# caizexin/GenVC

Measured on AMD Instinct MI355X. Metric: utterances/s (streaming, 1 s chunks; with RTF and first-chunk latency), higher is better.
Workload: dtype f32; 1 GPU; GenVC_small streaming, 1 s chunks, top_k=1, batch 1 per GPU (BASELINE configs[1]); parallelism=replicas x1, utterances sharded by rank, all_gather of token ids

## Files before the change

genvc_amd/csrc/gemm.h:

```cpp
#pragma once
#include "common.h"

namespace gvc {

__host__ __device__ __forceinline__ size_t fm16_index(int m, int k, int K) {
    return ((size_t)(m >> 4) * (K >> 4) + (k >> 4)) * 256 + (size_t)((((m & 15) + 16 * ((k & 15) >> 2)) << 2) + (k & 3));
}

enum GemmAct { ACT_NONE = 0, ACT_GELU_NEW = 1, ACT_RELU = 2, ACT_GELU_ERF = 3 };
enum GemmAAct { AACT_NONE = 0, AACT_LRELU = 1 };

struct GemmEpi {
    const float* bias;
    long long bias_batch_stride;
    int act;
    const float* resid;
    int ldr;
    long long resid_batch_stride;
    long long resid_batch_stride2;
    int resid_fm16;
    int geglu;
    const float* resid2;
    float out_scale;
    int c_fm16;
    int qkv;
    int d, n_head, head_dim, max_seq, T;
    float* kcache; float* vcache;
    int kv_bf16;
    const int32_t* slots;
    const int32_t* base_len;
};

struct GemmArgs {
    const float* A; int lda; long long a_batch_stride;
    const float* Wt; int ldw; long long w_batch_stride;
    int w_bf16;
    float* C; int ldc; long long c_batch_stride;
    int batch_inner; long long a_batch_stride2, c_batch_stride2;
    int M, N, K;
    int conv_cin, conv_tap_stride;
    int a_act; float a_slope;
    const float* att_part; int att_nc, att_heads, att_hd;
    int SK;
    float* work;
    GemmEpi e;
};

__device__ __forceinline__ long long gemm_boff(const GemmArgs& G, int batch, long long s1, long long s2) {
    return G.batch_inner > 0 ? (long long)(batch % G.batch_inner) * s1 + (long long)(batch / G.batch_inner) * s2 : (long long)batch * s1;
}
__device__ __forceinline__ int gemm_binner(const GemmArgs& G, int batch) { return G.batch_inner > 0 ? batch % G.batch_inner : batch; }

__device__ __forceinline__ void gemm_store_nb(const GemmArgs& G, int batch, int m, int n, float v) {
    const GemmEpi& e = G.e;
    if (e.act == ACT_GELU_NEW) v = gelu_new(v);
    else if (e.act == ACT_RELU) v = fmaxf(v, 0.f);
    else if (e.act == ACT_GELU_ERF) v = gelu_erf(v);
    if (e.qkv) {
        const int which = n / e.d;
        const int c = n - which * e.d;
        if (which == 0) {
            G.C[(size_t)m * G.ldc + c] = v;
        } else {
            const int b = m / e.T, t = m - b * e.T;
            const int slot = e.slots[b];
            const int pos = t + (e.base_len ? e.base_len[slot] : 0);
            const int h = c / e.head_dim, j = c - h * e.head_dim;
            float* cache = which == 1 ? e.kcache : e.vcache;
            const size_t at = (((size_t)slot * e.n_head + h) * e.max_seq + pos) * e.head_dim + j;
            if (e.kv_bf16) reinterpret_cast<unsigned short*>(cache)[at] = f32_to_bf16(v);
            else cache[at] = v;
        }
        return;
    }
    if (e.resid) v += e.resid[gemm_boff(G, batch, e.resid_batch_stride, e.resid_batch_stride2) + (size_t)m * e.ldr + n];
    if (e.resid2) v += e.resid2[gemm_boff(G, batch, e.resid_batch_stride, e.resid_batch_stride2) + (size_t)m * e.ldr + n];
    if (e.out_scale != 0.f) v *= e.out_scale;
    if (e.c_fm16) { G.C[fm16_index(m, n, G.N)] = v; return; }
    G.C[gemm_boff(G, batch, G.c_batch_stride, G.c_batch_stride2) + (size_t)m * G.ldc + n] = v;
}

__device__ __forceinline__ void gemm_store(const GemmArgs& G, int batch, int m, int n, float v) {
    if (G.e.bias) v += G.e.bias[gemm_binner(G, batch) * G.e.bias_batch_stride + n];
    gemm_store_nb(G, batch, m, n, v);
}

__device__ __forceinline__ void gemm_store4(const GemmArgs& G, int m, int n, float4 v) {
    const GemmEpi& e = G.e;
    if (e.bias) {
        const float4 b = *reinterpret_cast<const float4*>(e.bias + n);
        v.x += b.x; v.y += b.y; v.z += b.z; v.w += b.w;
    }
    if (e.act == ACT_GELU_NEW) { v.x = gelu_new(v.x); v.y = gelu_new(v.y); v.z = gelu_new(v.z); v.w = gelu_new(v.w); }
    else if (e.act == ACT_RELU) { v.x = fmaxf(v.x, 0.f); v.y = fmaxf(v.y, 0.f); v.z = fmaxf(v.z, 0.f); v.w = fmaxf(v.w, 0.f); }
    else if (e.act == ACT_GELU_ERF) { v.x = gelu_erf(v.x); v.y = gelu_erf(v.y); v.z = gelu_erf(v.z); v.w = gelu_erf(v.w); }
    if (e.qkv) {
        const int which = n / e.d;
        const int c = n - which * e.d;
        if (which == 0) {
            *reinterpret_cast<float4*>(G.C + (size_t)m * G.ldc + c) = v;
        } else {
            const int b = m / e.T, t = m - b * e.T;
            const int slot = e.slots[b];
            const int pos = t + (e.base_len ? e.base_len[slot] : 0);
            const int h = c / e.head_dim, j = c - h * e.head_dim;
            float* cache = which == 1 ? e.kcache : e.vcache;
            const size_t at = (((size_t)slot * e.n_head + h) * e.max_seq + pos) * e.head_dim + j;
            if (e.kv_bf16) {
                ushort4 o;
                o.x = f32_to_bf16(v.x); o.y = f32_to_bf16(v.y); o.z = f32_to_bf16(v.z); o.w = f32_to_bf16(v.w);
                *reinterpret_cast<ushort4*>(reinterpret_cast<unsigned short*>(cache) + at) = o;
// ... 128 lines not shown
```

genvc_amd/csrc/gpt.hip:

```cpp
#include <stdlib.h>

#include <map>
#include <string>
#include <tuple>
#include <vector>

#include "gemm.h"
#include <algorithm>
#include "gpt_kernels.h"
#include "persist_kernel.h"
#include "persist_rows.h"
#include "persist_rows_b16.h"
#include "beam.h"
#include "cfg.h"
#include "contrastive.h"
#include "sampler.h"
#include "seqscore.h"
#include "spec.h"

namespace gvc {

__global__ void k_ln_rows(const float* src, float* dst, int rows, int d, const float* w1, const float* b1,
                          const float* w2, const float* b2, int dst_fm16) {
    const int lane = threadIdx.x & 63;
// ... 1 lines not shown
    if (row >= rows) return;
    const float* x = src + (size_t)row * d;
    float* y = dst + (size_t)row * d;
    const float inv_d = 1.0f / (float)d;
    for (int pass = 0; pass < (w2 ? 2 : 1); ++pass) {
        const float* in = pass == 0 ? x : y;
        const float* gw = pass == 0 ? w1 : w2;
        const float* gb = pass == 0 ? b1 : b2;
        float s = 0.f;
        for (int k = lane * 4; k < d; k += 256) {
            const float4 v = *reinterpret_cast<const float4*>(in + k);
            s += (v.x + v.y) + (v.z + v.w);
        }
        const float mean = wave_sum(s) * inv_d;
        float q = 0.f;
        for (int k = lane * 4; k < d; k += 256) {
            const float4 v = *reinterpret_cast<const float4*>(in + k);
            const float a0 = v.x - mean, a1 = v.y - mean, a2 = v.z - mean, a3 = v.w - mean;
            q += (a0 * a0 + a1 * a1) + (a2 * a2 + a3 * a3);
        }
        const float rstd = 1.0f / sqrtf(wave_sum(q) * inv_d + 1e-5f);
        for (int k = lane * 4; k < d; k += 256) {
            float4 v = *reinterpret_cast<const float4*>(in + k);
            const float4 g = *reinterpret_cast<const float4*>(gw + k);
            const float4 c = *reinterpret_cast<const float4*>(gb + k);
            v.x = (v.x - mean) * rstd * g.x + c.x; v.y = (v.y - mean) * rstd * g.y + c.y;
            v.z = (v.z - mean) * rstd * g.z + c.z; v.w = (v.w - mean) * rstd * g.w + c.w;
            if (dst_fm16 && !w2) *reinterpret_cast<float4*>(dst + fm16_index(row, k, d)) = v;
            else *reinterpret_cast<float4*>(y + k) = v;
        }
    }
}

__global__ void k_embed_rows(float* x, const float* prefix_emb, int B, int T, int P, int d, const float* mel_emb,
                             const float* mel_pos, const int32_t* codes, int n, int start_tok, int stop_tok, int t_off) {
    const int row = blockIdx.x;
    const int Tn = T - t_off;
    const int b = row / Tn, t = row - b * Tn + t_off;
    float* dst = x + (size_t)row * d;
    if (t < P) {
        const float* src = prefix_emb + ((size_t)b * P + t) * d;
        for (int k = threadIdx.x * 4; k < d; k += blockDim.x * 4)
            *reinterpret_cast<float4*>(dst + k) = *reinterpret_cast<const float4*>(src + k);
    } else {
        const int i = t - P;
        const int tok = i == 0 ? start_tok : (i <= n ? codes[(size_t)b * n + i - 1] : stop_tok);
        const float* e = mel_emb + (size_t)tok * d;
        const float* p = mel_pos + (size_t)i * d;
        for (int k = threadIdx.x * 4; k < d; k += blockDim.x * 4) {
            const float4 a = *reinterpret_cast<const float4*>(e + k);
            const float4 c = *reinterpret_cast<const float4*>(p + k);
            *reinterpret_cast<float4*>(dst + k) = make_float4(a.x + c.x, a.y + c.y, a.z + c.z, a.w + c.w);
        }
    }
}

__global__ void k_prefix_rows(float* out, const float* cond, int n_cond, const int32_t* codes, int B, int Tc,
                              int d, const float* text_emb, const float* text_pos, int start_text,
                              int stop_text) {
    const int P = n_cond + Tc + 2;
    const int row = blockIdx.x;
    const int b = row / P, t = row - b * P;
    float* dst = out + (size_t)row * d;
    if (t < n_cond) {
        const float* src = cond + ((size_t)b * n_cond + t) * d;
        for (int k = threadIdx.x * 4; k < d; k += blockDim.x * 4)
            *reinterpret_cast<float4*>(dst + k) = *reinterpret_cast<const float4*>(src + k);
    } else {
        const int i = t - n_cond;
        const int id = i == 0 ? start_text : (i <= Tc ? codes[(size_t)b * Tc + i - 1] : stop_text);
        const float* e = text_emb + (size_t)id * d;
        const float* p = text_pos + (size_t)i * d;
        for (int k = threadIdx.x * 4; k < d; k += blockDim.x * 4) {
            const float4 a = *reinterpret_cast<const float4*>(e + k);
            const float4 c = *reinterpret_cast<const float4*>(p + k);
            *reinterpret_cast<float4*>(dst + k) = make_float4(a.x + c.x, a.y + c.y, a.z + c.z, a.w + c.w);
        }
    }
}

__global__ void k_embed_decode_rows(float* x, const int32_t* tok, const int32_t* slots, GptState st, const float* mel_emb,
                                    const float* mel_pos, int d, int vocab) {
    const int b = blockIdx.x;
    const float* e = mel_emb + (size_t)min(max(tok[b], 0), vocab - 1) * d;
    const float* p = mel_pos + (size_t)st.mel_pos[slots[b]] * d;
    float* dst = x + (size_t)b * d;
    for (int k = threadIdx.x * 4; k < d; k += blockDim.x * 4) {
        const float4 a = *reinterpret_cast<const float4*>(e + k);
        const float4 c = *reinterpret_cast<const float4*>(p + k);
        *reinterpret_cast<float4*>(dst + k) = make_float4(a.x + c.x, a.y + c.y, a.z + c.z, a.w + c.w);
    }
}

__global__ void k_stage_rows(float* stage, float* store, const int32_t* slots, int n, int to_store) {
    const int b = blockIdx.x;
    float* a = stage + (size_t)b * n;
    float* s = store + (size_t)slots[b] * n;
    for (int i = threadIdx.x; i < n; i += blockDim.x) {
        if (to_store) s[i] = a[i];
        else a[i] = s[i];
    }
}

__global__ void k_set_state(GptState st, const int32_t* slots, int B, int seq_len, int mel_pos) {
    const int b = blockIdx.x * blockDim.x + threadIdx.x;
    if (b < B) {
        st.seq_len[slots[b]] = seq_len;
        st.mel_pos[slots[b]] = mel_pos;
        st.pending[slots[b]] = -1;
    }
}

__global__ void k_gather_rows(const float* src, float* dst, int B, int T, int off, int n, int d) {
    const int row = blockIdx.x;
    const int b = row / n, i = row - b * n;
    const float* s = src + ((size_t)b * T + off + i) * d;
    float* o = dst + (size_t)row * d;
    for (int k = threadIdx.x * 4; k < d; k += blockDim.x * 4)
        *reinterpret_cast<float4*>(o + k) = *reinterpret_cast<const float4*>(s + k);
}

__global__ void k_round_bf16(float* w, unsigned short* out, size_t n) {
    for (size_t i = (size_t)blockIdx.x * blockDim.x + threadIdx.x; i < n; i += (size_t)gridDim.x * blockDim.x) {
        const unsigned u = __float_as_uint(w[i]);
        const unsigned r = u + 0x7fffu + ((u >> 16) & 1u);
        out[i] = (unsigned short)(r >> 16);
        w[i] = __uint_as_float(r & 0xffff0000u);
    }
}

__global__ void k_transpose(const float* src, float* dst, int K, int N) {
    __shared__ float tile[32][33];
    const int k0 = blockIdx.y * 32, n0 = blockIdx.x * 32;
    for (int r = threadIdx.y; r < 32; r += blockDim.y) {
        const int k = k0 + r, n = n0 + threadIdx.x;
        if (k < K && n < N) tile[r][threadIdx.x] = src[(size_t)k * N + n];
    }
    __syncthreads();
    for (int r = threadIdx.y; r < 32; r += blockDim.y) {
        const int n = n0 + r, k = k0 + threadIdx.x;
        if (k < K && n < N) dst[(size_t)n * K + k] = tile[threadIdx.x][r];
    }
}
// ... 1260 lines not shown
        G.A = c->h; G.lda = 4 * d; G.Wt = fm ? ly.p2_f : ly.p2_w; G.w_bf16 = fm && c->bf16; G.ldw = 4 * d; G.C = c->x; G.ldc = d; G.M = rows; G.N = d; G.K = 4 * d;
        if (fm) {
            G.work = part_p2;
            if ((rc = gemm_fm(G, strip ? 8 : SKP, 1, &sk_p2))) return rc;
        } else {
            G.work = c->work; G.e.bias = ly.p2_b; G.e.resid = c->x; G.e.ldr = d;
            if ((rc = launch_gemm_cap(G, 1, c->work_cap, s))) return rc;
        }
    }
    if (fm) {
        ln_sum_sk(part_p2, sk_p2, c->layers[c->dm.n_layer - 1].p2_b, nullptr, nullptr);
        GVC_LAUNCH_CHECK();
    }
    return ln_rc;
}

extern "C" int gvc_gpt_prefill(gvc_gpt* c, const int32_t* slots, int32_t B, const float* prefix_emb, int32_t P,
                               int32_t start_tok, float* logits_out, float* latent_out, gvc_stream sv) {
    return gvc_gpt_prefill_cached(c, slots, B, prefix_emb, P, 0, start_tok, logits_out, latent_out, sv);
}

static int prefill_impl(gvc_gpt* c, const int32_t* slots, int32_t B, const float* prefix_emb, int32_t P, int32_t n_cached,
                        int32_t start_tok, float* logits_out, float* latent_out, float* hidden_out, gvc_stream sv) {
    int rc = check_ready(c);
    if (rc) return rc;
    const int T = P + 1, d = c->dm.d_model;
    GVC_REQUIRE(n_cached >= 0 && n_cached <= P, GVC_ERR_ARG, "prefill: n_cached=%d outside [0,%d]", n_cached, P);
    GVC_REQUIRE(B >= 1 && B <= c->dm.max_slots, GVC_ERR_ARG, "prefill: B=%d outside [1,%d]", B, c->dm.max_slots);
    GVC_REQUIRE(P >= 0 && B * T <= c->dm.max_rows, GVC_ERR_ARG, "prefill: %d rows exceed max_rows %d", B * T, c->dm.max_rows);
    GVC_REQUIRE(T < c->dm.max_seq, GVC_ERR_ARG, "prefill: %d rows exceed max_seq %d", T, c->dm.max_seq);
    hipStream_t s = (hipStream_t)sv;
    if (!logits_out) logits_out = c->logits;
    if (!latent_out) latent_out = c->latent;
    hipLaunchKernelGGL(k_embed_rows, dim3(B * (T - n_cached)), dim3(256), 0, s, c->x, prefix_emb, B, T, P, d, c->mel_emb, c->mel_pos,
                       (const int32_t*)nullptr, 0, start_tok, start_tok, n_cached);
    GVC_LAUNCH_CHECK();
    const int Tn = T - n_cached;
    if (n_cached > 0 && rows_persist_ok(c, B * Tn, c->st.seq_len) && (rc = rows_persist_prepare(c))) return rc;
    c->rows_keys_hint = T;
    if (n_cached > 0) {
        hipLaunchKernelGGL(k_set_state, dim3(cdiv(B, 64)), dim3(64), 0, s, c->st, slots, B, n_cached, 0);
        GVC_LAUNCH_CHECK();
        if ((rc = run_rows(c, slots, B, Tn, s, c->st.seq_len))) return rc;
    } else if ((rc = run_rows(c, slots, B, T, s))) return rc;
    if (hidden_out) {
        hipLaunchKernelGGL(k_ln_rows, dim3(cdiv(B * Tn, 4)), dim3(256), 0, s, c->x, hidden_out, B * Tn, d, c->lnf_w, c->lnf_b,
                           (const float*)nullptr, (const float*)nullptr, 0);
        GVC_LAUNCH_CHECK();
    }
    if ((rc = launch_head(c, slots, B, 0, c->x, Tn, Tn - 1, logits_out, latent_out, 0, nullptr, s))) return rc;
    hipLaunchKernelGGL(k_set_state, dim3(cdiv(B, 64)), dim3(64), 0, s, c->st, slots, B, T, 1);
    GVC_LAUNCH_CHECK();
    hipLaunchKernelGGL(k_stage_rows, dim3(B), dim3(256), 0, s, logits_out, c->slot_logits, slots, c->dm.vocab, 1);
    hipLaunchKernelGGL(k_stage_rows, dim3(B), dim3(256), 0, s, latent_out, c->slot_latent, slots, d, 1);
    GVC_LAUNCH_CHECK();
    return GVC_OK;
}

extern "C" int gvc_gpt_prefill_cached(gvc_gpt* c, const int32_t* slots, int32_t B, const float* prefix_emb, int32_t P,
                                      int32_t n_cached, int32_t start_tok, float* logits_out, float* latent_out, gvc_stream sv) {
    return prefill_impl(c, slots, B, prefix_emb, P, n_cached, start_tok, logits_out, latent_out, nullptr, sv);
}

extern "C" int gvc_gpt_prefill_hidden(gvc_gpt* c, const int32_t* slots, int32_t B, const float* prefix_emb, int32_t P, int32_t start_tok,
                                      float* hidden_out, gvc_stream sv) {
    GVC_REQUIRE(hidden_out, GVC_ERR_ARG, "prefill_hidden: null hidden_out");
    return prefill_impl(c, slots, B, prefix_emb, P, 0, start_tok, nullptr, nullptr, hidden_out, sv);
}

extern "C" int gvc_gpt_prefill_cond(gvc_gpt* c, const int32_t* slots, int32_t B, const float* cond_latents, int32_t n_cond, gvc_stream sv) {
    int rc = check_ready(c);
    if (rc) return rc;
    const int d = c->dm.d_model;
    GVC_REQUIRE(B >= 1 && B <= c->dm.max_slots && n_cond >= 1 && B * n_cond <= c->dm.max_rows && n_cond < c->dm.max_seq, GVC_ERR_ARG,
                "prefill_cond: bad B=%d n_cond=%d", B, n_cond);
    hipStream_t s = (hipStream_t)sv;
    hipLaunchKernelGGL(k_embed_rows, dim3(B * n_cond), dim3(256), 0, s, c->x, cond_latents, B, n_cond, n_cond, d, c->mel_emb, c->mel_pos,
                       (const int32_t*)nullptr, 0, 0, 0, 0);
    GVC_LAUNCH_CHECK();
    c->rows_keys_hint = n_cond;
    if ((rc = run_rows(c, slots, B, n_cond, s))) return rc;
    hipLaunchKernelGGL(k_set_state, dim3(cdiv(B, 64)), dim3(64), 0, s, c->st, slots, B, n_cond, 0);
    GVC_LAUNCH_CHECK();
    return GVC_OK;
}

extern "C" int gvc_gpt_latents(gvc_gpt* c, const int32_t* slots, int32_t B, const float* prefix_emb, int32_t P,
// ... 865 lines not shown
```

genvc_amd/csrc/hubert.hip:

```cpp
#include <map>
#include <string>
#include <vector>

#include "conv_lds.h"
#include "attn64.h"
#include <algorithm>

namespace gvc {

constexpr int kC0Chunk = 32;

static __global__ void k_hb_repack_conv(const float* w, float* out, int Co, int Ci, int k) {
    const size_t n = (size_t)Co * Ci * k;
    for (size_t i = (size_t)blockIdx.x * blockDim.x + threadIdx.x; i < n; i += (size_t)gridDim.x * blockDim.x) {
        const int j = (int)(i % k);
        const int ci = (int)((i / k) % Ci);
        const int co = (int)(i / ((size_t)k * Ci));
        out[((size_t)co * k + j) * Ci + ci] = w[i];
    }
}

static __global__ __launch_bounds__(256) void k_hb_conv0(const float* wav, const float* w, float* y, float* part, int T,
                                                        int T0, int C, int k, int stride) {
    extern __shared__ float xs[];
    const int b = blockIdx.z, chunk = blockIdx.x, tid = threadIdx.x;
    const int t0 = chunk * kC0Chunk;
    const int nt = min(kC0Chunk, T0 - t0);
    const int nx = (nt - 1) * stride + k;
    const float* src = wav + (size_t)b * T + (size_t)t0 * stride;
    for (int i = tid; i < nx; i += 256) xs[i] = src[i];
    __syncthreads();
    for (int c = blockIdx.y * 256 + tid; c < min(C, (int)(blockIdx.y + 1) * 256); c += 256) {
        float wr[16];
#pragma unroll
        for (int j = 0; j < 16; ++j) wr[j] = j < k ? w[(size_t)c * k + j] : 0.f;
        float s = 0.f, ss = 0.f, a = 0.f;
        float* yo = y + ((size_t)b * T0 + t0) * C + c;
        for (int t = 0; t < nt; ++t) {
            float acc = 0.f;
#pragma unroll
            for (int j = 0; j < 16; ++j)
                if (j < k) acc = fmaf(wr[j], xs[t * stride + j], acc);
            yo[(size_t)t * C] = acc;
            if (t == 0) a = acc;
            const float dv = acc - a;
            s += dv; ss = fmaf(dv, dv, ss);
        }
        float* po = part + (((size_t)b * gridDim.x + chunk) * C + c) * 2;
        const float dm = s / (float)nt;
        po[0] = a + dm; po[1] = fmaxf(ss - s * dm, 0.f);
    }
}

static __global__ __launch_bounds__(256) void k_hb_gn_stats(const float* part, float* stats, int nchunk, int T0, int C) {
    const int b = blockIdx.y, c = blockIdx.x * 8 + (threadIdx.x >> 5), l = threadIdx.x & 31;
    if (c >= C) return;
    double s = 0.0, ss = 0.0;
    for (int i0 = l; i0 < nchunk; i0 += 32 * 8) {
        float2 pv[8];
#pragma unroll
        for (int u = 0; u < 8; ++u)
            pv[u] = *reinterpret_cast<const float2*>(part + (((size_t)b * nchunk + min(i0 + 32 * u, nchunk - 1)) * C + c) * 2);
#pragma unroll
        for (int u = 0; u < 8; ++u)
            if (i0 + 32 * u < nchunk) {
                const double n = (double)min(kC0Chunk, T0 - (i0 + 32 * u) * kC0Chunk), m = (double)pv[u].x;
                s += n * m; ss += (double)pv[u].y + n * m * m;
            }
    }
#pragma unroll
    for (int o = 16; o >= 1; o >>= 1) { s += __shfl_xor(s, o, 32); ss += __shfl_xor(ss, o, 32); }
    if (l) return;
    const double mean = s / T0;
    double var = ss / T0 - mean * mean;
    if (var < 0.0) var = 0.0;
    stats[((size_t)b * C + c) * 2] = (float)mean;
    stats[((size_t)b * C + c) * 2 + 1] = (float)(1.0 / sqrt(var + 1e-5));
}

static __global__ void k_hb_gn_gelu(float* y, const float* stats, const float* gamma, const float* beta, int T0, int C) {
    const int b = blockIdx.y;
    const size_t n4 = (size_t)T0 * C / 4;
    float* yb = y + (size_t)b * T0 * C;
    for (size_t i = (size_t)blockIdx.x * blockDim.x + threadIdx.x; i < n4; i += (size_t)gridDim.x * blockDim.x) {
        const int c = (int)((i * 4) % C);
        float4 v = *reinterpret_cast<float4*>(yb + i * 4);
        const float* st = stats + ((size_t)b * C + c) * 2;
        v.x = gelu_erf((v.x - st[0]) * st[1] * gamma[c] + beta[c]);
        v.y = gelu_erf((v.y - st[2]) * st[3] * gamma[c + 1] + beta[c + 1]);
        v.z = gelu_erf((v.z - st[4]) * st[5] * gamma[c + 2] + beta[c + 2]);
        v.w = gelu_erf((v.w - st[6]) * st[7] * gamma[c + 3] + beta[c + 3]);
        *reinterpret_cast<float4*>(yb + i * 4) = v;
    }
}

static __global__ __launch_bounds__(256) void k_hb_ln_rows(const float* src, long long src_bs, float* dst, long long dst_bs,
                                                          int rpb, int d, const float* w, const float* b,
                                                          const float* part = nullptr, int SK = 0, const float* pbias = nullptr,
                                                          int rows = 0, float* dst_fm16 = nullptr) {
    __shared__ float red[4];
    const int row = blockIdx.x, tid = threadIdx.x;
    const int bi = row / rpb, ri = row - bi * rpb;
    const float* xr = src + bi * src_bs + (size_t)ri * d;
    float* orow = dst + bi * dst_bs + (size_t)ri * d;
    float4 v[4];
    float s = 0.f;
#pragma unroll
    for (int i = 0; i < 4; ++i) {
        const int k = (i * 256 + tid) * 4;
        v[i] = k < d ? *reinterpret_cast<const float4*>(xr + k) : make_float4(0.f, 0.f, 0.f, 0.f);
        if (part && k < d) {
            const float4 b4 = *reinterpret_cast<const float4*>(pbias + k);
            float4 p4[8];
#pragma unroll
            for (int sidx = 0; sidx < 8; ++sidx)
                p4[sidx] = *reinterpret_cast<const float4*>(part + ((size_t)min(sidx, SK - 1) * rows + row) * d + k);
            v[i].x += b4.x; v[i].y += b4.y; v[i].z += b4.z; v[i].w += b4.w;
#pragma unroll
            for (int sidx = 0; sidx < 8; ++sidx)
                if (sidx < SK) { v[i].x += p4[sidx].x; v[i].y += p4[sidx].y; v[i].z += p4[sidx].z; v[i].w += p4[sidx].w; }
        }
        s += (v[i].x + v[i].y) + (v[i].z + v[i].w);
    }
    const float inv_d = 1.0f / (float)d;
    const float mean = block4_sum(s, red) * inv_d;
    float q = 0.f;
#pragma unroll
    for (int i = 0; i < 4; ++i) {
        const int k = (i * 256 + tid) * 4;
        if (k < d) {
            const float a0 = v[i].x - mean, a1 = v[i].y - mean, a2 = v[i].z - mean, a3 = v[i].w - mean;
            q += (a0 * a0 + a1 * a1) + (a2 * a2 + a3 * a3);
        }
    }
    const float rstd = 1.0f / sqrtf(block4_sum(q, red) * inv_d + 1e-5f);
#pragma unroll
    for (int i = 0; i < 4; ++i) {
        const int k = (i * 256 + tid) * 4;
        if (k < d) {
            const float4 gw = *reinterpret_cast<const float4*>(w + k);
            const float4 gb = *reinterpret_cast<const float4*>(b + k);
            float4 o;
            o.x = (v[i].x - mean) * rstd * gw.x + gb.x; o.y = (v[i].y - mean) * rstd * gw.y + gb.y;
            o.z = (v[i].z - mean) * rstd * gw.z + gb.z; o.w = (v[i].w - mean) * rstd * gw.w + gb.w;
            *reinterpret_cast<float4*>(orow + k) = o;
            if (dst_fm16) *reinterpret_cast<float4*>(dst_fm16 + fm16_index(row, k, d)) = o;
        }
    }
}

static __global__ void k_hb_zero_pad(float* buf, int C, int T, int front, int back, const int32_t* fmask) {
    const int b = blockIdx.y;
    float* base = buf + (size_t)b * (front + T + back) * C;
    const size_t nf = (size_t)front * C, nb = (size_t)back * C;
    for (size_t i = (size_t)blockIdx.x * blockDim.x + threadIdx.x; i < nf + nb; i += (size_t)gridDim.x * blockDim.x) {
        if (i < nf) base[i] = 0.f;
        else base[(size_t)(front + T) * C + (i - nf)] = 0.f;
    }
    for (int t = blockIdx.x; t < T; t += gridDim.x) {
        if (!fmask[b * T + t]) continue;
        for (int i = threadIdx.x; i < C; i += blockDim.x) base[(size_t)(front + t) * C + i] = 0.f;
    }
}

static __global__ __launch_bounds__(64) void k_hb_frame_mask(const float* wav, int32_t* fmask, int T, int F) {
    const int f = blockIdx.x, b = blockIdx.y, lane = threadIdx.x;
    const int chunk = T / F;
    const float* p = wav + (size_t)b * T + (size_t)f * chunk;
    int nz = 0;
    for (int i = lane; i < chunk; i += 64) nz |= (p[i] != 0.f);
    nz = __any(nz);
    if (lane == 0) fmask[b * F + f] = nz ? 0 : 1;
}

}

using namespace gvc;

struct HbLin { float* w = nullptr; float* b = nullptr; int N = 0, K = 0; float* wf = nullptr;  };
struct HbLn { float* w = nullptr; float* b = nullptr; };
struct HbLayer { HbLin qkv, out, fc1, fc2; HbLn ln1, ln2; };

struct gvc_hubert {
    gvc_hubert_dims dm;
    int cg = 0, pad_front = 0, pad_back = 0;
    float* conv0_w = nullptr;
    HbLn gn;
    std::vector<float*> conv_w;
    std::vector<float*> conv_wp;
    int conv_lds = 1;
    int conv_lds_rows = 256;
    HbLn feat_ln, enc_ln;
    HbLin proj, pos, fin;
    std::vector<HbLayer> layers;
    std::map<std::string, int> bound;
    int n_expected = 0;
    float *act[2] = {nullptr, nullptr};
    float *part = nullptr, *stats = nullptr;
    int32_t* fmask = nullptr;
    float *xp = nullptr, *x = nullptr, *qkv = nullptr, *att = nullptr, *hbuf = nullptr, *tmp = nullptr, *work = nullptr;
    long long work_cap = 0;
    int max_frames = 0, max_t0 = 0;
    std::map<long long, hipGraphExec_t> graphs;
    hipStream_t cap_stream = nullptr;
    int use_graph = 1;
    int skinny = 1;
    int strip = 1;
    bool fm_ready = false;
    float *xf = nullptr, *af = nullptr, *hf = nullptr;
    std::vector<void*> allocs;
};

static int hb_alloc(gvc_hubert* c, float** p, size_t n) {
    GVC_CHECK_HIP(hipMalloc((void**)p, n * sizeof(float)));
    c->allocs.push_back(*p);
    return GVC_OK;
}
static int hb_alloc_lin(gvc_hubert* c, HbLin& L, int N, int K) {
    L.N = N; L.K = K;
    int rc = hb_alloc(c, &L.w, (size_t)N * K);
    return rc ? rc : hb_alloc(c, &L.b, N);
}
static int hb_alloc_ln(gvc_hubert* c, HbLn& L, int d) {
    int rc = hb_alloc(c, &L.w, d);
    return rc ? rc : hb_alloc(c, &L.b, d);
}

static int hb_frames(const gvc_hubert_dims& D, int n, int upto) {
    for (int i = 0; i < upto; ++i) {
        if (n < D.conv_kernel[i]) return 0;
        n = (n - D.conv_kernel[i]) / D.conv_stride[i] + 1;
    }
// ... 155 lines not shown
        if (which >= 0) {
            if (is_b) rc = hb_copy(L.qkv.b + (size_t)which * E, src, numel, E, name, s);
            else rc = hb_copy(L.qkv.w + (size_t)which * E * E, src, numel, (int64_t)E * E, name, s);
        } else if (sub.rfind("self_attn.out_proj.", 0) == 0) rc = lin(L.out);
        else if (sub.rfind("self_attn_layer_norm.", 0) == 0) rc = ln(L.ln1, E);
        else if (sub.rfind("fc1.", 0) == 0) rc = lin(L.fc1);
        else if (sub.rfind("fc2.", 0) == 0) rc = lin(L.fc2);
        else if (sub.rfind("final_layer_norm.", 0) == 0) rc = ln(L.ln2, E);
        else known = false;
    } else known = false;
    if (rc == GVC_OK && known) { c->bound[n] = 1; c->fm_ready = false; }
    return rc;
}

extern "C" int gvc_hubert_missing_weights(gvc_hubert* c) { return c ? c->n_expected - (int)c->bound.size() : -1; }

static int hb_linear(gvc_hubert* c, const HbLin& L, const float* A, float* C, int M, int act, const float* resid, hipStream_t s) {
    GemmArgs G;
    memset(&G, 0, sizeof(G));
    G.A = A; G.lda = L.K; G.Wt = L.w; G.ldw = L.K; G.C = C; G.ldc = L.N;
    G.M = M; G.N = L.N; G.K = L.K; G.work = c->work;
    G.e.bias = L.b; G.e.act = act;
    if (resid) { G.e.resid = resid; G.e.ldr = L.N; }
    return launch_gemm_cap(G, 1, c->work_cap, s);
}

static int hb_body(gvc_hubert* c, int B, int T, hipStream_t s) {
    const gvc_hubert_dims& D = c->dm;
    const int E = D.embed_dim;
    int rc;
    int Tin = hb_frames(D, T, 1);
    const int C0 = D.conv_dim[0];
    const int nchunk = cdiv(Tin, kC0Chunk);
    hipLaunchKernelGGL(k_hb_gn_stats, dim3(cdiv(C0, 8), B), dim3(256), 0, s, c->part, c->stats, nchunk, Tin, C0);
    GVC_LAUNCH_CHECK();
    {
        const size_t n4 = (size_t)Tin * C0 / 4;
        const int gx = (int)std::min<size_t>((n4 + 255) / 256, 4096);
        hipLaunchKernelGGL(k_hb_gn_gelu, dim3(gx, B), dim3(256), 0, s, c->act[0], c->stats, c->gn.w, c->gn.b, Tin, C0);
        GVC_LAUNCH_CHECK();
    }
    int cur = 0;
    for (int i = 1; i < D.n_conv; ++i) {
        const int Ci = D.conv_dim[i - 1], Co = D.conv_dim[i], k = D.conv_kernel[i], st = D.conv_stride[i];
        const int Tout = (Tin - k) / st + 1;
        if (c->conv_lds && c->conv_wp[i - 1] && Tout <= c->conv_lds_rows) {
            ConvLdsArgs A;
            memset(&A, 0, sizeof(A));
            A.x = c->act[cur]; A.x_bs = (long long)Tin * Ci; A.ldx = Ci; A.x_scale = 1.f; A.slope = 1.f;
            A.x_rows = Tin; A.stride = st;
            A.y = c->act[cur ^ 1]; A.y_bs = (long long)Tout * Co; A.ldy = Co;
            A.T = Tout; A.ntiles = Co / 16; A.act = ACT_GELU_ERF;
            A.job[0].wp = reinterpret_cast<const float4*>(c->conv_wp[i - 1]); A.job[0].k = k; A.job[0].dil = 1;
            if ((rc = launch_conv_lds(Ci, 1, A, 1, B, conv_lds_bytes(Ci, k, 1, false, st), s))) return rc;
            cur ^= 1;
            Tin = Tout;
            continue;
        }
        GemmArgs G;
        memset(&G, 0, sizeof(G));
        G.A = c->act[cur]; G.lda = st * Ci; G.a_batch_stride = (long long)Tin * Ci;
        G.Wt = c->conv_w[i - 1]; G.ldw = k * Ci;
        G.C = c->act[cur ^ 1]; G.ldc = Co; G.c_batch_stride = (long long)Tout * Co;
        G.M = Tout; G.N = Co; G.K = k * Ci; G.work = c->work;
        G.e.act = ACT_GELU_ERF;
        if ((rc = launch_gemm_cap(G, B, c->work_cap, s))) return rc;
        cur ^= 1;
        Tin = Tout;
    }
    const int F = Tin, Cl = D.conv_dim[D.n_conv - 1], rows = B * F;
    const int kp = D.pos_conv_kernel;
    const long long xp_bs = (long long)(F + kp - 1) * E;
    hipLaunchKernelGGL(k_hb_ln_rows, dim3(rows), dim3(256), 0, s, c->act[cur], (long long)F * Cl, c->act[cur ^ 1],
                       (long long)F * Cl, F, Cl, c->feat_ln.w, c->feat_ln.b);
    GVC_LAUNCH_CHECK();
    {
        GemmArgs G;
        memset(&G, 0, sizeof(G));
        G.A = c->act[cur ^ 1]; G.lda = Cl; G.a_batch_stride = (long long)F * Cl;
        G.Wt = c->proj.w; G.ldw = Cl;
        G.C = c->xp + (size_t)c->pad_front * E; G.ldc = E; G.c_batch_stride = xp_bs;
        G.M = F; G.N = E; G.K = Cl; G.work = c->work;
        G.e.bias = c->proj.b;
        if ((rc = launch_gemm_cap(G, B, c->work_cap, s))) return rc;
    }
    hipLaunchKernelGGL(k_hb_zero_pad, dim3(64, B), dim3(256), 0, s, c->xp, E, F, c->pad_front, c->pad_back, c->fmask);
    GVC_LAUNCH_CHECK();
    {
        GemmArgs G;
        memset(&G, 0, sizeof(G));
        const int cg = c->cg;
        G.batch_inner = D.pos_conv_groups;
        G.A = c->xp; G.lda = E; G.a_batch_stride = cg; G.a_batch_stride2 = xp_bs;
        G.conv_cin = cg; G.conv_tap_stride = E;
        G.Wt = c->pos.w; G.ldw = kp * cg; G.w_batch_stride = (long long)cg * kp * cg;
        G.C = c->tmp; G.ldc = E; G.c_batch_stride = cg; G.c_batch_stride2 = (long long)F * E;
        G.M = F; G.N = cg; G.K = kp * cg; G.work = c->work;
        G.e.bias = c->pos.b; G.e.bias_batch_stride = cg; G.e.act = ACT_GELU_ERF;
        G.e.resid = c->xp + (size_t)c->pad_front * E; G.e.ldr = E; G.e.resid_batch_stride = cg; G.e.resid_batch_stride2 = xp_bs;
        if ((rc = launch_gemm_cap(G, B * D.pos_conv_groups, c->work_cap, s))) return rc;
    }
    const bool skinny = c->skinny && (rows <= 128 || (c->strip && E % 64 == 0 && D.ffn_dim % 64 == 0));
    const bool strip = rows > 128;
    if (skinny) {
        hipLaunchKernelGGL(k_hb_ln_rows, dim3(rows), dim3(256), 0, s, c->tmp, (long long)F * E, c->x, (long long)F * E, F, E,
                           c->enc_ln.w, c->enc_ln.b, (const float*)nullptr, 0, (const float*)nullptr, rows, c->xf);
        GVC_LAUNCH_CHECK();
        int sk_used = 1;
        auto sk_gemm = [&](const HbLin& L, const float* A_fm, float* C, int act, int c_fm16, int SK, const float* resid = nullptr) {
            GemmArgs G;
            memset(&G, 0, sizeof(G));
            G.A = A_fm; G.lda = L.K; G.Wt = L.wf; G.ldw = L.K; G.C = C; G.ldc = L.N; G.M = rows; G.N = L.N; G.K = L.K;
            G.work = c->work;
            if (strip && resid) {
                if ((long long)rows * L.N > c->work_cap) { set_error("hubert: %d rows exceed the split-K work buffer", rows); return (int)GVC_ERR_ARG; }
                return launch_gemm_strip(G, 8, c->work_cap, 1, &sk_used, s);
            }
            sk_used = SK;
            if (SK == 1) { G.e.bias = L.b; G.e.act = act; G.e.c_fm16 = c_fm16; G.e.resid = resid; G.e.ldr = L.N; }
            if (strip) return launch_gemm_strip(G, 1, c->work_cap, 0, nullptr, s);
// ... 33 lines not shown
        hipLaunchKernelGGL(k_attn64_mfma<true>, dim3(cdiv(F, 16), D.n_heads, B), dim3(256), 0, s, c->qkv, c->qkv + E, c->qkv + 2 * E, (long long)3 * E, (long long)F * 3 * E, F, F, c->att, F, E, 0.125f, 0, c->fmask);
        GVC_LAUNCH_CHECK();
        if ((rc = hb_linear(c, L.out, c->att, c->tmp, rows, ACT_NONE, c->x, s))) return rc;
        hipLaunchKernelGGL(k_hb_ln_rows, dim3(rows), dim3(256), 0, s, c->tmp, (long long)F * E, c->x, (long long)F * E, F, E,
                           L.ln1.w, L.ln1.b);
        GVC_LAUNCH_CHECK();
        if ((rc = hb_linear(c, L.fc1, c->x, c->hbuf, rows, ACT_GELU_ERF, nullptr, s))) return rc;
        if ((rc = hb_linear(c, L.fc2, c->hbuf, c->tmp, rows, ACT_NONE, c->x, s))) return rc;
        hipLaunchKernelGGL(k_hb_ln_rows, dim3(rows), dim3(256), 0, s, c->tmp, (long long)F * E, c->x, (long long)F * E, F, E,
                           L.ln2.w, L.ln2.b);
        GVC_LAUNCH_CHECK();
    }
    return GVC_OK;
}

extern "C" int gvc_hubert_forward(gvc_hubert* c, const float* wav, int32_t B, int32_t T, float* out, gvc_stream sv) {
    GVC_REQUIRE(c && wav && out, GVC_ERR_ARG, "gvc_hubert_forward: null argument");
    GVC_REQUIRE(gvc_hubert_missing_weights(c) == 0, GVC_ERR_STATE, "%d HuBERT weight tensors are not bound",
                gvc_hubert_missing_weights(c));
    const gvc_hubert_dims& D = c->dm;
    const int F = hb_frames(D, T, D.n_conv);
    GVC_REQUIRE(B >= 1 && B <= D.max_batch && T <= D.max_samples && F >= 1, GVC_ERR_ARG,
                "hubert: B=%d samples=%d outside capacity (%d, %d) or too short", B, T, D.max_batch, D.max_samples);
    hipStream_t s = (hipStream_t)sv;
    if (c->skinny && !c->fm_ready) {
        for (HbLayer& L : c->layers)
            for (HbLin* q : {&L.qkv, &L.out, &L.fc1, &L.fc2}) {
                hipLaunchKernelGGL(k_to_fm16, dim3(1024), dim3(256), 0, s, q->w, q->wf, q->N, q->K);
                GVC_LAUNCH_CHECK();
            }
        c->fm_ready = true;
    }
    const int T0 = hb_frames(D, T, 1), C0 = D.conv_dim[0], k0 = D.conv_kernel[0], s0 = D.conv_stride[0];
    hipLaunchKernelGGL(k_hb_conv0, dim3(cdiv(T0, kC0Chunk), cdiv(C0, 256), B), dim3(256), ((kC0Chunk - 1) * s0 + k0) * sizeof(float), s, wav,
                       c->conv0_w, c->act[0], c->part, T, T0, C0, k0, s0);
    GVC_LAUNCH_CHECK();
    hipLaunchKernelGGL(k_hb_frame_mask, dim3(F, B), dim3(64), 0, s, wav, c->fmask, T, F);
    GVC_LAUNCH_CHECK();
    int rc;
    if (!c->use_graph) {
        if ((rc = hb_body(c, B, T, s))) return rc;
    } else {
        const long long key = ((long long)B << 32) | (unsigned)T;
        auto it = c->graphs.find(key);
        if (it == c->graphs.end()) {
            if (c->graphs.size() >= 64) {
                for (auto& kv : c->graphs) hipGraphExecDestroy(kv.second);
                c->graphs.clear();
            }
            hipGraphExec_t ge;
            if ((rc = capture_graph(c->cap_stream, &ge, [&] { return hb_body(c, B, T, c->cap_stream); }))) return rc;
            it = c->graphs.emplace(key, ge).first;
        }
        GVC_CHECK_HIP(hipGraphLaunch(it->second, s));
    }
    {
        GemmArgs G;
        memset(&G, 0, sizeof(G));
        const HbLin& L = c->fin;
        G.A = c->x; G.lda = L.K; G.Wt = L.w; G.ldw = L.K; G.C = out; G.ldc = L.N;
        G.M = B * F; G.N = L.N; G.K = L.K; G.work = c->work;
        G.e.bias = L.b;
        if ((rc = launch_gemm_cap(G, 1, c->work_cap, s))) return rc;
    }
    return GVC_OK;
}
```

Measured before the change: 7.038 utterances/s.

## Fuse small HuBERT and GPT prefill kernels to cut launch count

Several small kernels are merged. The frame mask is folded into the conv0 launch as extra blocks, GroupNorm stats and GELU become one kernel, and pad zeroing moves into the projection GEMM epilogue (a row_zero mask) plus a one-time memset of the padded buffer when B or F changes. In GPT prefill, the embedding and set-state kernels are combined, and set-state plus the two staging copies become one park kernel. This trims launch overhead and memory passes on the streaming path, at the risk of correctness if the pad regions are ever dirtied between calls with the same shape.

Result: no change. 7.051 utterances/s (median of 2 runs) (+0.2%).

```diff
diff --git a/genvc_amd/csrc/gemm.h b/genvc_amd/csrc/gemm.h
--- a/genvc_amd/csrc/gemm.h
+++ b/genvc_amd/csrc/gemm.h
@@ -29,6 +29,7 @@
     int kv_bf16;
     const int32_t* slots;
     const int32_t* base_len;
+    const int32_t* row_zero;
 };
 
 struct GemmArgs {
@@ -77,6 +78,7 @@
     if (e.resid2) v += e.resid2[gemm_boff(G, batch, e.resid_batch_stride, e.resid_batch_stride2) + (size_t)m * e.ldr + n];
     if (e.out_scale != 0.f) v *= e.out_scale;
     if (e.c_fm16) { G.C[fm16_index(m, n, G.N)] = v; return; }
+    if (e.row_zero && e.row_zero[(size_t)batch * G.M + m]) v = 0.f;
     G.C[gemm_boff(G, batch, G.c_batch_stride, G.c_batch_stride2) + (size_t)m * G.ldc + n] = v;
 }
 
diff --git a/genvc_amd/csrc/gpt.hip b/genvc_amd/csrc/gpt.hip
--- a/genvc_amd/csrc/gpt.hip
+++ b/genvc_amd/csrc/gpt.hip
@@ -57,9 +57,8 @@
     }
 }
 
-__global__ void k_embed_rows(float* x, const float* prefix_emb, int B, int T, int P, int d, const float* mel_emb,
-                             const float* mel_pos, const int32_t* codes, int n, int start_tok, int stop_tok, int t_off) {
-    const int row = blockIdx.x;
+__device__ __forceinline__ void embed_row(int row, float* x, const float* prefix_emb, int T, int P, int d, const float* mel_emb,
+                                          const float* mel_pos, const int32_t* codes, int n, int start_tok, int stop_tok, int t_off) {
     const int Tn = T - t_off;
     const int b = row / Tn, t = row - b * Tn + t_off;
     float* dst = x + (size_t)row * d;
@@ -78,6 +77,26 @@
             *reinterpret_cast<float4*>(dst + k) = make_float4(a.x + c.x, a.y + c.y, a.z + c.z, a.w + c.w);
         }
     }
+}
+
+__global__ void k_embed_rows(float* x, const float* prefix_emb, int B, int T, int P, int d, const float* mel_emb,
+                             const float* mel_pos, const int32_t* codes, int n, int start_tok, int stop_tok, int t_off) {
+    embed_row(blockIdx.x, x, prefix_emb, T, P, d, mel_emb, mel_pos, codes, n, start_tok, stop_tok, t_off);
+}
+
+__device__ __forceinline__ void set_slot_state(const GptState& st, int slot, int seq_len, int mel_pos) {
+    st.seq_len[slot] = seq_len;
+    st.mel_pos[slot] = mel_pos;
+    st.pending[slot] = -1;
+}
+
+__global__ void k_embed_rows_state(float* x, const float* prefix_emb, int rows, int T, int P, int d, const float* mel_emb,
+                                   const float* mel_pos, int start_tok, int t_off, GptState st, const int32_t* slots, int B) {
+    if ((int)blockIdx.x == rows) {
+        for (int b = threadIdx.x; b < B; b += blockDim.x) set_slot_state(st, slots[b], t_off, 0);
+        return;
+    }
+    embed_row(blockIdx.x, x, prefix_emb, T, P, d, mel_emb, mel_pos, nullptr, 0, start_tok, start_tok, t_off);
 }
 
 __global__ void k_prefix_rows(float* out, const float* cond, int n_cond, const int32_t* codes, int B, int Tc,
@@ -129,11 +148,15 @@
 
 __global__ void k_set_state(GptState st, const int32_t* slots, int B, int seq_len, int mel_pos) {
     const int b = blockIdx.x * blockDim.x + threadIdx.x;
-    if (b < B) {
-        st.seq_len[slots[b]] = seq_len;
-        st.mel_pos[slots[b]] = mel_pos;
-        st.pending[slots[b]] = -1;
-    }
+    if (b < B) set_slot_state(st, slots[b], seq_len, mel_pos);
+}
+
+__global__ void k_prefill_park(GptState st, const int32_t* slots, int seq_len, int mel_pos, const float* logits, float* slot_logits,
+                               int vocab, const float* latent, float* slot_latent, int d) {
+    const int b = blockIdx.x, slot = slots[b];
+    if (threadIdx.x == 0) set_slot_state(st, slot, seq_len, mel_pos);
+    for (int i = threadIdx.x; i < vocab; i += blockDim.x) slot_logits[(size_t)slot * vocab + i] = logits[(size_t)b * vocab + i];
+    for (int i = threadIdx.x; i < d; i += blockDim.x) slot_latent[(size_t)slot * d + i] = latent[(size_t)b * d + i];
 }
 
 __global__ void k_gather_rows(const float* src, float* dst, int B, int T, int off, int n, int d) {
@@ -1460,27 +1483,28 @@
     hipStream_t s = (hipStream_t)sv;
     if (!logits_out) logits_out = c->logits;
     if (!latent_out) latent_out = c->latent;
-    hipLaunchKernelGGL(k_embed_rows, dim3(B * (T - n_cached)), dim3(256), 0, s, c->x, prefix_emb, B, T, P, d, c->mel_emb, c->mel_pos,
-                       (const int32_t*)nullptr, 0, start_tok, start_tok, n_cached);
-    GVC_LAUNCH_CHECK();
     const int Tn = T - n_cached;
     if (n_cached > 0 && rows_persist_ok(c, B * Tn, c->st.seq_len) && (rc = rows_persist_prepare(c))) return rc;
     c->rows_keys_hint = T;
     if (n_cached > 0) {
-        hipLaunchKernelGGL(k_set_state, dim3(cdiv(B, 64)), dim3(64), 0, s, c->st, slots, B, n_cached, 0);
+        hipLaunchKernelGGL(k_embed_rows_state, dim3(B * Tn + 1), dim3(256), 0, s, c->x, prefix_emb, B * Tn, T, P, d, c->mel_emb, c->mel_pos,
+                           start_tok, n_cached, c->st, slots, B);
         GVC_LAUNCH_CHECK();
         if ((rc = run_rows(c, slots, B, Tn, s, c->st.seq_len))) return rc;
-    } else if ((rc = run_rows(c, slots, B, T, s))) return rc;
+    } else {
+        hipLaunchKernelGGL(k_embed_rows, dim3(B * T), dim3(256), 0, s, c->x, prefix_emb, B, T, P, d, c->mel_emb, c->mel_pos,
+                           (const int32_t*)nullptr, 0, start_tok, start_tok, 0);
+        GVC_LAUNCH_CHECK();
+        if ((rc = run_rows(c, slots, B, T, s))) return rc;
+    }
     if (hidden_out) {
         hipLaunchKernelGGL(k_ln_rows, dim3(cdiv(B * Tn, 4)), dim3(256), 0, s, c->x, hidden_out, B * Tn, d, c->lnf_w, c->lnf_b,
                            (const float*)nullptr, (const float*)nullptr, 0);
         GVC_LAUNCH_CHECK();
     }
     if ((rc = launch_head(c, slots, B, 0, c->x, Tn, Tn - 1, logits_out, latent_out, 0, nullptr, s))) return rc;
-    hipLaunchKernelGGL(k_set_state, dim3(cdiv(B, 64)), dim3(64), 0, s, c->st, slots, B, T, 1);
-    GVC_LAUNCH_CHECK();
-    hipLaunchKernelGGL(k_stage_rows, dim3(B), dim3(256), 0, s, logits_out, c->slot_logits, slots, c->dm.vocab, 1);
-    hipLaunchKernelGGL(k_stage_rows, dim3(B), dim3(256), 0, s, latent_out, c->slot_latent, slots, d, 1);
+    hipLaunchKernelGGL(k_prefill_park, dim3(B), dim3(256), 0, s, c->st, slots, T, 1, logits_out, c->slot_logits, c->dm.vocab, latent_out,
+                       c->slot_latent, d);
     GVC_LAUNCH_CHECK();
     return GVC_OK;
 }
diff --git a/genvc_amd/csrc/hubert.hip b/genvc_amd/csrc/hubert.hip
--- a/genvc_amd/csrc/hubert.hip
+++ b/genvc_amd/csrc/hubert.hip
@@ -20,10 +20,17 @@
     }
 }
 
+static __device__ __forceinline__ void hb_frame_mask(const float* wav, int32_t* fmask, int T, int F, int f, int b, int lane);
 static __global__ __launch_bounds__(256) void k_hb_conv0(const float* wav, const float* w, float* y, float* part, int T,
-                                                        int T0, int C, int k, int stride) {
+                                                        int T0, int C, int k, int stride, int nchunk, int32_t* fmask, int F) {
     extern __shared__ float xs[];
     const int b = blockIdx.z, chunk = blockIdx.x, tid = threadIdx.x;
+    if (chunk >= nchunk) {
+        if (blockIdx.y) return;
+        const int f = (chunk - nchunk) * 4 + (tid >> 6);
+        if (f < F) hb_frame_mask(wav, fmask, T, F, f, b, tid & 63);
+        return;
+    }
     const int t0 = chunk * kC0Chunk;
     const int nt = min(kC0Chunk, T0 - t0);
     const int nx = (nt - 1) * stride + k;
@@ -46,15 +53,13 @@
             const float dv = acc - a;
             s += dv; ss = fmaf(dv, dv, ss);
         }
-        float* po = part + (((size_t)b * gridDim.x + chunk) * C + c) * 2;
+        float* po = part + (((size_t)b * nchunk + chunk) * C + c) * 2;
         const float dm = s / (float)nt;
         po[0] = a + dm; po[1] = fmaxf(ss - s * dm, 0.f);
     }
 }
 
-static __global__ __launch_bounds__(256) void k_hb_gn_stats(const float* part, float* stats, int nchunk, int T0, int C) {
-    const int b = blockIdx.y, c = blockIdx.x * 8 + (threadIdx.x >> 5), l = threadIdx.x & 31;
-    if (c >= C) return;
+static __device__ __forceinline__ float2 hb_gn_channel_stats(const float* part, int nchunk, int T0, int C, int b, int c, int l) {
     double s = 0.0, ss = 0.0;
     for (int i0 = l; i0 < nchunk; i0 += 32 * 8) {
         float2 pv[8];
@@ -70,12 +75,19 @@
     }
 #pragma unroll
     for (int o = 16; o >= 1; o >>= 1) { s += __shfl_xor(s, o, 32); ss += __shfl_xor(ss, o, 32); }
-    if (l) return;
     const double mean = s / T0;
     double var = ss / T0 - mean * mean;
     if (var < 0.0) var = 0.0;
-    stats[((size_t)b * C + c) * 2] = (float)mean;
-    stats[((size_t)b * C + c) * 2 + 1] = (float)(1.0 / sqrt(var + 1e-5));
+    return make_float2((float)mean, (float)(1.0 / sqrt(var + 1e-5)));
+}
+
+static __global__ __launch_bounds__(256) void k_hb_gn_stats(const float* part, float* stats, int nchunk, int T0, int C) {
+    const int b = blockIdx.y, c = blockIdx.x * 8 + (threadIdx.x >> 5), l = threadIdx.x & 31;
+    if (c >= C) return;
+    const float2 st = hb_gn_channel_stats(part, nchunk, T0, C, b, c, l);
+    if (l) return;
+    stats[((size_t)b * C + c) * 2] = st.x;
+    stats[((size_t)b * C + c) * 2 + 1] = st.y;
 }
 
 static __global__ void k_hb_gn_gelu(float* y, const float* stats, const float* gamma, const float* beta, int T0, int C) {
@@ -94,6 +106,32 @@
     }
 }
 
+constexpr int kGnRows = 256;
+static __global__ __launch_bounds__(256) void k_hb_gn_stats_gelu(float* y, const float* part, const float* gamma, const float* beta,
+                                                                int nchunk, int T0, int C) {
+    __shared__ float st_s[32 * 2];
+    const int b = blockIdx.z, c0 = blockIdx.x * 32, tid = threadIdx.x;
+#pragma unroll
+    for (int pass = 0; pass < 4; ++pass) {
+        const int ci = pass * 8 + (tid >> 5);
+        const float2 st = hb_gn_channel_stats(part, nchunk, T0, C, b, c0 + ci, tid & 31);
+        if ((tid & 31) == 0) { st_s[ci * 2] = st.x; st_s[ci * 2 + 1] = st.y; }
+    }
+    __syncthreads();
+    const int c = c0 + (tid & 7) * 4;
+    const float* st = st_s + (tid & 7) * 8;
+    const int t_end = min(T0, (int)(blockIdx.y + 1) * kGnRows);
+    for (int t = blockIdx.y * kGnRows + (tid >> 3); t < t_end; t += 32) {
+        float* p = y + ((size_t)b * T0 + t) * C + c;
+        float4 v = *reinterpret_cast<float4*>(p);
+        v.x = gelu_erf((v.x - st[0]) * st[1] * gamma[c] + beta[c]);
+        v.y = gelu_erf((v.y - st[2]) * st[3] * gamma[c + 1] + beta[c + 1]);
+        v.z = gelu_erf((v.z - st[4]) * st[5] * gamma[c + 2] + beta[c + 2]);
+        v.w = gelu_erf((v.w - st[6]) * st[7] * gamma[c + 3] + beta[c + 3]);
+        *reinterpret_cast<float4*>(p) = v;
+    }
+}
+
 static __global__ __launch_bounds__(256) void k_hb_ln_rows(const float* src, long long src_bs, float* dst, long long dst_bs,
                                                           int rpb, int d, const float* w, const float* b,
                                                           const float* part = nullptr, int SK = 0, const float* pbias = nullptr,
@@ -149,22 +187,7 @@
     }
 }
 
-static __global__ void k_hb_zero_pad(float* buf, int C, int T, int front, int back, const int32_t* fmask) {
-    const int b = blockIdx.y;
-    float* base = buf + (size_t)b * (front + T + back) * C;
-    const size_t nf = (size_t)front * C, nb = (size_t)back * C;
-    for (size_t i = (size_t)blockIdx.x * blockDim.x + threadIdx.x; i < nf + nb; i += (size_t)gridDim.x * blockDim.x) {
-        if (i < nf) base[i] = 0.f;
-        else base[(size_t)(front + T) * C + (i - nf)] = 0.f;
-    }
-    for (int t = blockIdx.x; t < T; t += gridDim.x) {
-        if (!fmask[b * T + t]) continue;
-        for (int i = threadIdx.x; i < C; i += blockDim.x) base[(size_t)(front + t) * C + i] = 0.f;
-    }
-}
-
-static __global__ __launch_bounds__(64) void k_hb_frame_mask(const float* wav, int32_t* fmask, int T, int F) {
-    const int f = blockIdx.x, b = blockIdx.y, lane = threadIdx.x;
+static __device__ __forceinline__ void hb_frame_mask(const float* wav, int32_t* fmask, int T, int F, int f, int b, int lane) {
     const int chunk = T / F;
     const float* p = wav + (size_t)b * T + (size_t)f * chunk;
     int nz = 0;
@@ -198,6 +221,7 @@
     float *act[2] = {nullptr, nullptr};
     float *part = nullptr, *stats = nullptr;
     int32_t* fmask = nullptr;
+    int xp_B = 0, xp_F = 0;
     float *xp = nullptr, *x = nullptr, *qkv = nullptr, *att = nullptr, *hbuf = nullptr, *tmp = nullptr, *work = nullptr;
     long long work_cap = 0;
     int max_frames = 0, max_t0 = 0;
@@ -419,9 +443,13 @@
     int Tin = hb_frames(D, T, 1);
     const int C0 = D.conv_dim[0];
     const int nchunk = cdiv(Tin, kC0Chunk);
-    hipLaunchKernelGGL(k_hb_gn_stats, dim3(cdiv(C0, 8), B), dim3(256), 0, s, c->part, c->stats, nchunk, Tin, C0);
-    GVC_LAUNCH_CHECK();
-    {
+    if (C0 % 32 == 0) {
+        hipLaunchKernelGGL(k_hb_gn_stats_gelu, dim3(C0 / 32, cdiv(Tin, kGnRows), B), dim3(256), 0, s, c->act[0], c->part, c->gn.w, c->gn.b,
+                           nchunk, Tin, C0);
+        GVC_LAUNCH_CHECK();
+    } else {
+        hipLaunchKernelGGL(k_hb_gn_stats, dim3(cdiv(C0, 8), B), dim3(256), 0, s, c->part, c->stats, nchunk, Tin, C0);
+        GVC_LAUNCH_CHECK();
         const size_t n4 = (size_t)Tin * C0 / 4;
         const int gx = (int)std::min<size_t>((n4 + 255) / 256, 4096);
         hipLaunchKernelGGL(k_hb_gn_gelu, dim3(gx, B), dim3(256), 0, s, c->act[0], c->stats, c->gn.w, c->gn.b, Tin, C0);
@@ -469,10 +497,9 @@
         G.C = c->xp + (size_t)c->pad_front * E; G.ldc = E; G.c_batch_stride = xp_bs;
         G.M = F; G.N = E; G.K = Cl; G.work = c->work;
         G.e.bias = c->proj.b;
+        G.e.row_zero = c->fmask;
         if ((rc = launch_gemm_cap(G, B, c->work_cap, s))) return rc;
     }
-    hipLaunchKernelGGL(k_hb_zero_pad, dim3(64, B), dim3(256), 0, s, c->xp, E, F, c->pad_front, c->pad_back, c->fmask);
-    GVC_LAUNCH_CHECK();
     {
         GemmArgs G;
         memset(&G, 0, sizeof(G));
@@ -572,10 +599,13 @@
         c->fm_ready = true;
     }
     const int T0 = hb_frames(D, T, 1), C0 = D.conv_dim[0], k0 = D.conv_kernel[0], s0 = D.conv_stride[0];
-    hipLaunchKernelGGL(k_hb_conv0, dim3(cdiv(T0, kC0Chunk), cdiv(C0, 256), B), dim3(256), ((kC0Chunk - 1) * s0 + k0) * sizeof(float), s, wav,
-                       c->conv0_w, c->act[0], c->part, T, T0, C0, k0, s0);
-    GVC_LAUNCH_CHECK();
-    hipLaunchKernelGGL(k_hb_frame_mask, dim3(F, B), dim3(64), 0, s, wav, c->fmask, T, F);
+    if (B != c->xp_B || F != c->xp_F) {
+        GVC_CHECK_HIP(hipMemsetAsync(c->xp, 0, (size_t)B * (F + D.pos_conv_kernel - 1) * D.embed_dim * sizeof(float), s));
+        c->xp_B = B; c->xp_F = F;
+    }
+    const int nchunk = cdiv(T0, kC0Chunk);
+    hipLaunchKernelGGL(k_hb_conv0, dim3(nchunk + cdiv(F, 4), cdiv(C0, 256), B), dim3(256), ((kC0Chunk - 1) * s0 + k0) * sizeof(float), s, wav,
+                       c->conv0_w, c->act[0], c->part, T, T0, C0, k0, s0, nchunk, c->fmask, F);
     GVC_LAUNCH_CHECK();
     int rc;
     if (!c->use_graph) {
```
